# huangeddie/GymGo

Measured on AMD Instinct MI355X. Metric: env steps/sec across batched games, 19x19 uniform-random rollouts, higher is better.
Workload: dtype u8; 1 GPU; 19x19, 65536 parallel games, uniform-random rollouts with auto-reset; one bench step = one launch of 256 plies for every game; board=19, games=65536, games_per_gpu=65536, env_steps_per_bench_step=16777216, burn_in_steps=1, desync_plies=640

## Files before the change

gymgo_amd/csrc/gg_v5.h:

```cpp
#pragma once
#include "gg_v4.h"

namespace gg {

constexpr int kNB5 = 32;
constexpr int kJobCap = 128;

template <int R>
struct Lds5 {
  static constexpr int RS = R == 13 ? 20 : Cfg<R>::kRowStride;
  static constexpr int RPL = (R + 1) / 2;
  static_assert(2 * RPL <= RS, "a pair's rows must fit the row stride");
  static constexpr int kPad = 4;
  static constexpr int kState = kPad;
  static constexpr int kMeta = kState + 2 * kNB5 * RS;
  static constexpr int kFair = kMeta + 5 * kNB5;
  static constexpr int kTmp = kFair + 16;
  static constexpr int kUnion = kTmp + 4 * RS;
  static constexpr int kZero = kJobCap, kDump = kJobCap + 1;
  static constexpr int kCls = kUnion;
  static constexpr int kJob = kCls + kJobCap + 4;
  static constexpr int kG = kJob + kJobCap + 4;
  static constexpr int kSc = kG + 2 * kNB5 * RS;
  static constexpr int kLoopEnd = kSc + kWave * RS;
  static constexpr int kV2 = kUnion;
  static constexpr int kIoEnd = kV2 + (Lds2<R>::kRegion0 > 768 ? Lds2<R>::kRegion0 : 768);
  static constexpr int kDmaWords = (((kNB5 * (5 * R + 1) * 4 + 12 + 15) / 16 + kWave - 1) / kWave) * 256;
  static constexpr int kDmaEnd = kUnion + kDmaWords;
  static constexpr int kGrpBits = kUnion;
  static constexpr int kGrpWords = ((15 + kNB5 * 6 * R * R + 31) / 32 + 4) & ~3;
  static constexpr int kGrpLut = kGrpBits + kGrpWords;
  static constexpr int kGrpEnd = kGrpLut + 512;
  static constexpr int kMax2(int a, int b) { return a > b ? a : b; }
  static constexpr int kTotal = kMax2(kMax2(kLoopEnd, kIoEnd), kMax2(kDmaEnd, kGrpEnd));
  static_assert(kTotal * 4 <= 20480, "two waves per SIMD: 20 KB of LDS per wave");
  static_assert(kUnion % 4 == 0 && kG % 4 == 0 && kSc % 4 == 0, "16-byte alignment of the flood blocks");
  static_assert(3 * kNB5 * RS <= kLoopEnd - kUnion, "parked tracked rows fit the loop area");
};

__device__ __forceinline__ uint32_t mbcnt64(uint64_t m) {
  return __builtin_amdgcn_mbcnt_hi((uint32_t)(m >> 32), __builtin_amdgcn_mbcnt_lo((uint32_t)m, 0u));
}
constexpr int QP_L0 = 0xA0;

__device__ __forceinline__ void kth_set_bit10(const uint32_t (&v)[10], const uint32_t (&p)[10], uint32_t tt, int &rr, uint32_t &pos) {
  uint32_t ntt = ~tt;
  const uint32_t g5 = (uint32_t)((int32_t)(p[4] + ntt) >> 31);
  uint32_t a[5], t[4];
#pragma unroll
  for (int i = 0; i < 5; ++i) a[i] = B3(g5, v[5 + i], v[i], T_SEL);
#pragma unroll
  for (int i = 0; i < 4; ++i) t[i] = B3(g5, p[5 + i], p[i], T_SEL);
  uint32_t base = g5 & p[4], row = g5 & 5u;
  const uint32_t g2 = (uint32_t)((int32_t)(t[1] + ntt) >> 31);
  const uint32_t b0 = B3(g2, a[2], a[0], T_SEL), b1 = B3(g2, a[3], a[1], T_SEL), u0 = B3(g2, t[2], t[0], T_SEL);
  base = B3(g2, t[1], base, T_SEL);
  row = B3(g2, 2u, row, T_ANDOR);
  const uint32_t g1 = (uint32_t)((int32_t)(u0 + ntt) >> 31);
  uint32_t vr = B3(g1, b1, b0, T_SEL);
  base = B3(g1, u0, base, T_SEL);
  row -= g1;
  const uint32_t g1b = B3(g2, g1, (uint32_t)((int32_t)(t[3] + ntt) >> 31), TA & TB & TC);
  vr = B3(g1b, a[4], vr, T_SEL);
  base = B3(g1b, t[3], base, T_SEL);
  row -= g1b;
  ntt += base;
  uint32_t ps = 0;
#pragma unroll
  for (int sh = 16; sh >= 1; sh >>= 1) {
    const uint32_t e = (uint32_t)__popc((vr >> ps) & ((1u << sh) - 1u)) + ntt;
    const uint32_t ge = (uint32_t)((int32_t)e >> 31);
    ntt = B3(ge, e, ntt, T_SEL);
    ps = B3((uint32_t)sh, ge, ps, T_ANDOR);
  }
  rr = (int)row;
  pos = ps;
}

template <int R>
constexpr int flood_first_test() {
#ifdef GG_AB_FLOODK
  return R == 19 ? GG_AB_FLOODK : 3;
#else
  return R == 19 ? 2 : 3;
#endif
}

#ifdef GG_AB_SWEEPS
static __device__ unsigned long long gg_sweeps5[10];
#endif

#ifndef GG_AB_LIBSUM
#define GG_AB_LIBSUM 1
#endif
#ifndef GG_AB_PEEL
#define GG_AB_PEEL 1
#endif
#ifndef GG_AB_PRIO
#define GG_AB_PRIO 1
#endif
#ifndef GG_AB_PRIO_HAND
#define GG_AB_PRIO_HAND 0
#endif
#ifndef GG_AB_HAND1
#define GG_AB_HAND1 1
#endif

#ifndef GG_AB_MOVE_RC
#define GG_AB_MOVE_RC 1
#endif

template <int R>
__device__ __forceinline__ uint32_t job_liberties(const uint32_t (&gt)[R], const uint32_t (&ot)[R], const uint32_t (&m)[R]) {
  constexpr uint32_t FULLROW = (1u << R) - 1u;
  static_assert(R < 27, "the sum of R rows below 2^R stays inside 32 bits");
  auto row = [&](int r) -> uint32_t {
    const uint32_t e = B3(ot[r], m[r], FULLROW, ~(TA | TB) & TC & 0xFF);
    const uint32_t up = r > 0 ? gt[r - 1] : 0u, dn = r + 1 < R ? gt[r + 1] : 0u;
    const uint32_t dd = B3(shl1(gt[r]), gt[r] >> 1, up, T_OR3);
    return B3(dd, dn, e, (TA | TB) & TC);
  };
#if GG_AB_LIBSUM
  uint32_t o3[3] = {0u, 0u, 0u}, s3[3] = {0u, 0u, 0u};
  if (R & 1) o3[0] = s3[0] = row(0);
#pragma unroll
  for (int r = R & 1; r < R; r += 2) {
    const int c = (r / 2) % 3;
    const uint32_t la = row(r), lb = row(r + 1);
    o3[c] = la | lb | o3[c];
    s3[c] = la + lb + s3[c];
  }
  const uint32_t o = o3[0] | o3[1] | o3[2], s = s3[0] + s3[1] + s3[2];
  const uint32_t two = B3(o, 0u - o, s, (TA & TB) ^ TC);
#else
  uint32_t o3[3] = {0u, 0u, 0u}, d3[3] = {0u, 0u, 0u};
#pragma unroll
  for (int r = 0; r < R; ++r) {
    const uint32_t l = row(r);
    d3[r % 3] = B3(l, o3[r % 3], d3[r % 3], T_ANDOR);
    o3[r % 3] = B3(l, o3[r % 3], 0u, T_OR3);
  }
  const uint32_t o = B3(o3[0], o3[1], o3[2], T_OR3);
  const uint32_t d = B3(d3[0], d3[1], d3[2], T_OR3) | B3(o3[0], o3[1], o3[2], T_MAJ);
  const uint32_t two = B3(o - 1u, o, d, T_ANDOR);
#endif
  return (o != 0u ? 1u : 0u) + (two != 0u ? 1u : 0u);
}

template <int R, bool WEAK>
__device__ __forceinline__ void flood_jobs_restart(const uint32_t (&m)[R], const uint32_t (&mrev)[R], uint32_t (&f)[R], uint32_t (&res)[R],
                                           bool need, const uint32_t (&mm)[R], uint32_t &open) {
  int sweeps = 0;
#pragma unroll 1
  for (int it = 0; it < R * R; ++it) {
#pragma unroll
    for (int r = 0; r < R; ++r) FLOOD_VISIT(r, r - 1, (r & 1) != 0);
    if (it > 0) {
      uint32_t op = 0, opw = 0, pend = 0, above = 0;
#pragma unroll
      for (int r = R - 1; r >= 0; --r) {
        const uint32_t g = ((r + 1) & 1) ? __brev(f[r]) : f[r];
        res[r] = g;
        if (r < R - 1) {
          const uint32_t t = B3(above, m[r], g, T_AND_ANDN);
          if (WEAK) { op |= t; opw = B3(t, mm[r], opw, (TA & ~TB & 0xFF) | TC); }
          else or_pairs(op, pend, (R - 2 - r) & 1, t);
        }
        above = g;
      }
      if (!WEAK && ((R - 1) & 1)) op |= pend;
      open = op;
      if (__ballot((WEAK ? opw : op) != 0 && need) == 0) { sweeps = 2 * it + 1; break; }
    }
#pragma unroll
    for (int r = R - 1; r >= 0; --r) FLOOD_VISIT(r, r + 1, ((r + 1) & 1) != 0);
    if (it > 0) {
      uint32_t op = 0, opw = 0, pend = 0, below = 0;
#pragma unroll
      for (int r = 0; r < R; ++r) {
        const uint32_t g = (r & 1) ? __brev(f[r]) : f[r];
        res[r] = g;
        if (r > 0) {
          const uint32_t t = B3(below, m[r], g, T_AND_ANDN);
          if (WEAK) { op |= t; opw = B3(t, mm[r], opw, (TA & ~TB & 0xFF) | TC); }
          else or_pairs(op, pend, (r - 1) & 1, t);
        }
        below = g;
      }
      if (!WEAK && ((R - 1) & 1)) op |= pend;
      open = op;
      if (__ballot((WEAK ? opw : op) != 0 && need) == 0) { sweeps = 2 * it + 2; break; }
    }
  }
  (void)sweeps;
}

template <int R>
__device__ __forceinline__ uint32_t flood_jobs(const uint32_t (&m)[R], const uint32_t (&mrev)[R], uint32_t (&f)[R], uint32_t (&res)[R],
                                               const uint32_t (&ot)[R], const uint32_t (&mm)[R], bool isG, bool have) {
  constexpr int K = flood_first_test<R>();
  static_assert(K >= 1 && K <= 3, "the first closure test comes after one, two or three sweeps");
  uint32_t cnt = 0;
  bool resumed = false;
#ifdef GG_AB_SWEEPS
  int sw_ = 0, sw0_ = 0;
  uint32_t ng_ = 0, no_ = 0;
#define GG_SW5_SWEEP() (++sw_)
#else
#define GG_SW5_SWEEP() ((void)0)
#endif
  auto done = [&](uint32_t op, uint32_t opw) -> bool {
    if (!resumed && __ballot(opw != 0u && isG) != 0) return false;
    cnt = job_liberties<R>(res, ot, m);
    const bool unsettled = have && op != 0u && cnt < 2u;
    const uint64_t u = __ballot(unsettled);
#ifdef GG_AB_SWEEPS
    if (!resumed) { sw0_ = sw_; ng_ = (uint32_t)__popcll(__ballot(unsettled && isG)); no_ = (uint32_t)__popcll(u) - ng_; }
#endif
    resumed = true;
    return u == 0;
  };
  auto sweep_down = [&]() {
#pragma unroll
    for (int r = 0; r < R; ++r) FLOOD_VISIT(r, r - 1, (r & 1) != 0);
    GG_SW5_SWEEP();
  };
  auto sweep_up = [&]() {
#pragma unroll
    for (int r = R - 1; r >= 0; --r) FLOOD_VISIT(r, r + 1, ((r + 1) & 1) != 0);
    GG_SW5_SWEEP();
  };
  auto done_after_down = [&]() -> bool {
    uint32_t op = 0, opw = 0, above = 0;
#pragma unroll
    for (int r = R - 1; r >= 0; --r) {
      const uint32_t g = ((r + 1) & 1) ? __brev(f[r]) : f[r];
      res[r] = g;
      if (r < R - 1) {
        const uint32_t t = B3(above, m[r], g, T_AND_ANDN);
        op |= t;
        opw = B3(t, mm[r], opw, (TA & ~TB & 0xFF) | TC);
      }
      above = g;
    }
    return done(op, opw);
  };
  auto done_after_up = [&]() -> bool {
    uint32_t op = 0, opw = 0, below = 0;
#pragma unroll
    for (int r = 0; r < R; ++r) {
      const uint32_t g = (r & 1) ? __brev(f[r]) : f[r];
      res[r] = g;
      if (r > 0) {
        const uint32_t t = B3(below, m[r], g, T_AND_ANDN);
        op |= t;
        opw = B3(t, mm[r], opw, (TA & ~TB & 0xFF) | TC);
      }
      below = g;
    }
    return done(op, opw);
  };
  constexpr bool PEEL = GG_AB_PEEL != 0 && K == 2;
  bool fin = false;
  if constexpr (PEEL) {
    sweep_down();
    sweep_up();
    fin = done_after_up();
  }
  if (!fin) {
#pragma unroll 1
    for (int it = PEEL ? 1 : 0; it < R * R; ++it) {
      sweep_down();
      if ((PEEL || K <= 1 || it > 0) && done_after_down()) break;
      sweep_up();
      if ((PEEL || K <= 2 || it > 0) && done_after_up()) break;
    }
  }
#undef GG_SW5_SWEEP
#ifdef GG_AB_SWEEPS
  { int l_; asm volatile("v_mbcnt_lo_u32_b32 %0, -1, 0\n\tv_mbcnt_hi_u32_b32 %0, -1, %0" : "=v"(l_));
    if (l_ == 0) {
      const int ex_ = sw_ - sw0_;
      atomicAdd(&gg_sweeps5[0], (unsigned long long)sw0_); atomicAdd(&gg_sweeps5[1], 1ull);
      if (ng_ + no_) { atomicAdd(&gg_sweeps5[2], 1ull); atomicAdd(&gg_sweeps5[2 + (ex_ < 4 ? ex_ : 4)], 1ull); }
      atomicAdd(&gg_sweeps5[7], (unsigned long long)ng_); atomicAdd(&gg_sweeps5[8], (unsigned long long)no_);
      atomicAdd(&gg_sweeps5[9], (unsigned long long)ex_);
    } }
#endif
  return cnt;
}

#ifdef GG_AB_P3
static __device__ unsigned long long gg_p3[10];
#define GG_P3(k, n) (p3c_[k] += (n))
#else
#define GG_P3(k, n) ((void)0)
#endif
#ifdef GG_AB_MARK
#define GG_MARK(k) asm volatile("; GGMARK " #k ::: "memory")
#else
#define GG_MARK(k) do {} while (0)
#endif
#if defined(GG_AB_P3) || defined(GG_AB_LIVE)
#define GG_LIVE_CHECK 1
static __device__ unsigned long long gg_live_bad;
#endif

#ifdef GG_AB_WS
static __device__ unsigned long long gg_wsc[2];
#define GG_WSC_DECL uint32_t wsc_[2] = {0u, 0u}
#define GG_WSC(hit) (wsc_[(hit) ? 0 : 1] += 1u)
#define GG_WSC_FLUSH do { if (ws && ln0 == 0) { atomicAdd(&gg_wsc[0], (unsigned long long)wsc_[0]); \
    atomicAdd(&gg_wsc[1], (unsigned long long)wsc_[1]); } } while (0)
#else
#define GG_WSC_DECL do {} while (0)
#define GG_WSC(hit) ((void)0)
#define GG_WSC_FLUSH do {} while (0)
#endif
#ifdef GG_AB_LOADSPLIT
static __device__ unsigned long long gg_lsplit[4];
#define GG_LS_DECL unsigned long long tls_[3] = {0, 0, 0}, tlc_ = clock64()
#define GG_LS(k) do { asm volatile("s_waitcnt lgkmcnt(0)" ::: "memory"); __builtin_amdgcn_sched_barrier(0); \
    const unsigned long long n_ = clock64(); __builtin_amdgcn_sched_barrier(0); tls_[k] += n_ - tlc_; tlc_ = n_; } while (0)
#define GG_LS_START do { __builtin_amdgcn_sched_barrier(0); tlc_ = clock64(); __builtin_amdgcn_sched_barrier(0); } while (0)
#define GG_LS_FLUSH do { if (ln0 == 0) { for (int k_ = 0; k_ < 3; ++k_) atomicAdd(&gg_lsplit[k_], tls_[k_]); \
    atomicAdd(&gg_lsplit[3], 1ull); } } while (0)
#else
// ... 24 lines not shown
```

gymgo_amd/csrc/gg_v5_kernel.h:

```cpp
template <int R, int IO>
__global__ __launch_bounds__(kWave, 2) void GG_R5_NAME(uint8_t *__restrict__ states, uint64_t *__restrict__ rng,
                                                       int32_t *__restrict__ last_actions, int64_t *__restrict__ steps_done,
                                                       int64_t B, uint32_t inv, int plies, int auto_reset, int nb,
                                                       uint32_t *__restrict__ ws) {
  constexpr int POL = GG_R5_POL;
  static_assert(IO == 0 || IO == 2, "byte planes or tracked boards");
  constexpr int N = R;
  constexpr int RS = Lds5<R>::RS;
  constexpr int RV = (R + 3) / 4;
  constexpr int RPL = Lds5<R>::RPL;
  constexpr int PL = kNB5 * RS;
  constexpr int ZERO = Lds5<R>::kZero, DUMP = Lds5<R>::kDump;
  constexpr bool TRACKED = IO == 2;
  constexpr int P = N * N, S = 6 * P, W = 5 * N + 1;
  constexpr uint32_t FULLROW = (1u << N) - 1u;
  __shared__ __attribute__((aligned(16))) uint32_t lds[Lds5<R>::kTotal];
  uint32_t *st = lds + Lds5<R>::kState;
  uint32_t *flagsv = lds + Lds5<R>::kMeta;
  int *lastv = reinterpret_cast<int *>(lds + Lds5<R>::kMeta + kNB5);
  int *playedv = reinterpret_cast<int *>(lds + Lds5<R>::kMeta + 2 * kNB5);
  uint32_t *rngv = lds + Lds5<R>::kMeta + 3 * kNB5;
  uint32_t *tmp = lds + Lds5<R>::kTmp;
  uint32_t *clsv = lds + Lds5<R>::kCls;
  uint32_t *jobv = lds + Lds5<R>::kJob;
// ... 149 lines not shown
        if (!known) {
          uint32_t ab;
          analyze2<R, false>(black, white, hf.full_l1 & ~(black | white), hf, v2, mb, ab, mw, nullptr, nullptr, true);
        }
        GG_LS(1);
        if (row) {
          st[0 * PL + s * RS + hf.hl] = black;
          st[1 * PL + s * RS + hf.hl] = white;
          tmp[(hf.h * 2 + 0) * RS + hf.hl] = invalid;
          tmp[(hf.h * 2 + 1) * RS + hf.hl] = mb | mw;
        }
        if (hf.hl == 0) {
          flagsv[s] = turn | (passed << 1) | (done << 2) | (on ? 8u : 0u);
          lastv[s] = -1;
          playedv[s] = 0;
        }
        WAVE_SYNC();
        if ((hf.lane >> 2) == i) {
          const uint32_t *tp = tmp + ((s5 & 1) * 2) * RS + r05;
#pragma unroll
          for (int r = 0; r < RPL; ++r) {
            inv_r[r] = tp[r];
            M[r] = tp[RS + r];
          }
        }
        WAVE_SYNC();
        GG_LS(2);
        cv0 = nv0; cv1 = nv1; cv2 = nv2; cfb = nfb;
        if (ws) { cw0 = nw0; cw1 = nw1; cw2 = nw2; cw3 = nw3; }
      }
#undef GG_ISSUE_PAIR5
#undef GG_ISSUE_WS5
      GG_LS_FLUSH;
    }
    WAVE_SYNC();
    for (int i = hf.lane; i < kWave * RS; i += kWave) sc[i] = 0u;
    WAVE_SYNC();

    uint32_t flr = flagsv[s5];
    const uint64_t x0r = ((uint64_t)rngv[2 * s5 + 1] << 32) | rngv[2 * s5];
    int playedr = 0;
#ifdef GG_AB_P3
    uint32_t p3c_[10] = {0, 0, 0, 0, 0, 0, 0, 0, 0, 0};
#endif
#ifdef GG_LIVE_CHECK
    int drawsr = 0;
    bool was_dead = false;
#endif
    GG_PROF(6);
    FairShare fair(lds + Lds5<R>::kFair);
    const uint32_t fair_lag = plies >= 192 ? 24u : (plies >= 16 ? (uint32_t)plies >> 3 : 2u);
    bool lead = false;
    uint32_t uq = 0;
#pragma unroll 1
    for (int t = 0; t < plies; ++t) {
      if ((t & 3) == 0 && plies >= 8) {
        const uint32_t left = (uint32_t)(plies - t);
        lead = fair.behind((uint32_t)t, left < fair_lag ? (left > 2u ? left : 2u) : fair_lag) != 0u;
        if (lead) __builtin_amdgcn_s_setprio(2); else __builtin_amdgcn_s_setprio(3);
      }
      int ln;
      asm volatile("v_mbcnt_lo_u32_b32 %0, -1, 0\n\tv_mbcnt_hi_u32_b32 %0, -1, %0" : "=v"(ln));
      const int s4 = (ln >> 1) & 31, t5 = ln & 1, r0 = RPL * t5;
      const bool bl = s4 < nb;
      uint32_t full[RPL];
#pragma unroll
      for (int r = 0; r < RPL; ++r) full[r] = (r0 + r < N) ? FULLROW : 0u;

      int a_q;
      uint32_t fl_q;
#if GG_AB_MOVE_RC
      uint32_t rc_q;
#endif
      {
        const uint32_t fl = flr;
        const bool on = bl && ((fl >> 3) & 1u);
        const bool done = (fl >> 2) & 1u;
        const bool live = on && !(done && !auto_reset);
        const bool reset = live && done;
#ifdef GG_LIVE_CHECK
        if (live && was_dead) atomicAdd(&gg_live_bad, 1ull);
        was_dead = was_dead || (bl && !live);
        drawsr += live ? 1 : 0;
#endif
        uint32_t v[RPL], p[RPL];
        const uint32_t rm = reset ? ~0u : 0u;
        uint32_t eye[RPL];
        uint32_t tc[RPL], te[RPL];
        if constexpr (POL != kPolUniform) {
          const uint32_t turn = fl & 1u;
          const uint32_t *pm = st + turn * PL + s4 * RS + r0, *po = st + (1u - turn) * PL + s4 * RS + r0;
          uint32_t me[RPL], op[RPL];
#pragma unroll
          for (int r = 0; r < RPL; ++r) { me[r] = pm[r]; op[r] = po[r]; }
          const uint32_t me_up = dpp0<QP_X1>(me[RPL - 1]), op_up = dpp0<QP_X1>(op[RPL - 1]);
          const uint32_t me_dn = dpp0<QP_X1>(me[0]), op_dn = dpp0<QP_X1>(op[0]);
          uint32_t m_up = 0u, m_dn = 0u;
          if constexpr (POL == kPolTactical) { m_up = dpp0<QP_X1>(M[RPL - 1]); m_dn = dpp0<QP_X1>(M[0]); }
#pragma unroll
          for (int r = 0; r < RPL; ++r) {
            const int rw = r0 + r;
            const uint32_t meU = r ? me[r - 1] : (t5 ? me_up : FULLROW), opU = r ? op[r - 1] : (t5 ? op_up : 0u);
            const uint32_t meDn = r + 1 < RPL ? me[r + 1] : (t5 ? 0u : me_dn), opD = r + 1 < RPL ? op[r + 1] : (t5 ? 0u : op_dn);
            const uint32_t meD = rw + 1 >= N ? FULLROW : meDn;
            const uint32_t edge = (rw == 0 || rw == N - 1) ? FULLROW : (1u | (1u << (N - 1)));
            eye[r] = eye_row(me[r], op[r], meU, meD, opU, opD, full[r], edge, N) & ~rm;
            if constexpr (POL == kPolTactical) {
              const uint32_t MU = r ? M[r - 1] : (t5 ? m_up : FULLROW);
              const uint32_t MDn = r + 1 < RPL ? M[r + 1] : (t5 ? 0u : m_dn);
              const uint32_t MD = rw + 1 >= N ? FULLROW : MDn;
              tactical_rows(me[r], op[r], M[r], meU, meD, opU, opD, MU, MD, full[r], tc[r], te[r]);
              tc[r] &= ~rm;
              te[r] &= ~rm;
            }
          }
        }
#pragma unroll
        for (int r = 0; r < RPL; ++r) {
          v[r] = B3(full[r], rm, inv_r[r], TA & (TB | (~TC & 0xFF)));
          if constexpr (POL == kPolTactical) {
            tc[r] &= v[r];
            te[r] &= v[r];
            v[r] &= ~eye[r];
            p[r] = ((uint32_t)__popc(v[r]) | ((uint32_t)__popc(tc[r]) << 10) | ((uint32_t)__popc(te[r]) << 20)) + (r ? p[r - 1] : 0u);
          } else {
            if constexpr (POL == kPolNoEyeFill) v[r] &= ~eye[r];
            p[r] = (uint32_t)__popc(v[r]) + (r ? p[r - 1] : 0u);
          }
        }
        uint32_t T = p[RPL - 1];
        const uint32_t oth = dpp0<QP_X1>(T);
        uint32_t Pb = t5 ? oth : 0u, n = T + oth;
        if ((t & 1) == 0) {
          uint64_t xx = x0r + (uint64_t)(uint32_t)(t + t5) * 0x9E3779B97F4A7C15ull;
          uq = (uint32_t)(splitmix_next(xx) >> 32);
        }
        const uint32_t uh = dpp0<QP_L0>(uq);
        uq = dpp0<QP_X1>(uq);
        if constexpr (POL == kPolTactical) {
          const bool gate = (uh & 3u) != 0u;
          const bool useC = gate && ((n >> 10) & 0x3FFu) != 0u, useE = gate && !useC && (n >> 20) != 0u;
          const uint32_t sh = useC ? 10u : (useE ? 20u : 0u);
          const uint32_t mc = useC ? ~0u : 0u, me_ = useE ? ~0u : 0u;
#pragma unroll
          for (int r = 0; r < RPL; ++r) {
            v[r] = B3(mc, tc[r], B3(me_, te[r], v[r], T_SEL), T_SEL);
            p[r] = (p[r] >> sh) & 0x3FFu;
          }
          T = (T >> sh) & 0x3FFu;
          Pb = (Pb >> sh) & 0x3FFu;
          n = (n >> sh) & 0x3FFu;
        }
        const uint32_t k = __umulhi(uh, POL != kPolUniform ? n : n + 1u);
        const bool hit = k >= Pb && k < Pb + T;
        int rr;
        uint32_t pos;
        if constexpr (RPL == 10) kth_set_bit10(v, p, (k - Pb) & 0x3FFu, rr, pos);
        else kth_set_bit<RPL>(v, p, (k - Pb) & 0x3FFu, rr, pos);
        const int rabs = r0 + rr;
#if GG_AB_MOVE_RC
        const uint32_t cand = hit ? ((uint32_t)rabs << 5) | pos : 0u;
        rc_q = cand | dpp0<QP_X1>(cand);
        const uint32_t pt = __umul24(rc_q >> 5, (uint32_t)N) + (rc_q & 31u);
#else
        const uint32_t cand = hit ? (uint32_t)(rabs * N + (int)pos) : 0u;
        const uint32_t pt = cand | dpp0<QP_X1>(cand);
#endif
        a_q = !live ? -1 : (k < n ? (int)pt : P);
        const bool place = live && hit;
        fl_q = reset ? 40u : fl;
        uint64_t resetm = __ballot(reset && t5 == 0);
        const bool none_live = __ballot(live) == 0;
        if (none_live && resetm == 0) break;
        if (resetm) {
          if (reset) {
#pragma unroll
            for (int r = 0; r < RPL; ++r) inv_r[r] = M[r] = 0u;
          }
          while (resetm) {
            const int s = (__ffsll((unsigned long long)resetm) - 1) >> 1;
            resetm &= resetm - 1;
            for (int i = hf.lane; i < 2 * RS; i += kWave) st[(i / RS) * PL + s * RS + (i % RS)] = 0;
            if (hf.lane == 0) flagsv[s] = 8u | 32u;
          }
          if (none_live) break;
        }
        WAVE_SYNC();
        uint32_t *gb = gblk + 2 * s4 * RS;
        if (t5 == 0) clsv[s4] = 0u;
        {
          uint4 *pz = reinterpret_cast<uint4 *>(gb + t5 * RS);
#pragma unroll
          for (int i = 0; i < RV; ++i) pz[i] = make_uint4(0u, 0u, 0u, 0u);
        }
        asm volatile("" ::: "memory");
        if (place) {
          const int turn = reset ? 0 : (int)(fl & 1u);
          atomicOr(st + turn * PL + s4 * RS + rabs, 1u << pos);
          gb[rabs] = 1u << pos;
        }
      }
      WAVE_SYNC();
      GG_PROF(0);

      uint32_t qs;
      int njobs;
      {
        const int a = a_q;
        const uint32_t turn = fl_q & 1u;
        const uint32_t mv1 = ((uint32_t)a < (uint32_t)P) ? 1u : 0u;
        int ar, ac;
#if GG_AB_MOVE_RC
        ar = (int)(rc_q >> 5);
        ac = (int)(rc_q & 31u);
#else
        split_action(mv1 ? a : 0, N, inv, ar, ac);
#endif
        const uint32_t *pm = st + turn * PL + s4 * RS, *po = st + (1u - turn) * PL + s4 * RS;
        uint32_t obit[2], packed = 0;
#pragma unroll
        for (int j = 0; j < 2; ++j) {
          const int sg = 2 * j - 1;
          const int dr = t5 ? 0 : sg, dc = t5 ? sg : 0;
          const int nr = ar + dr, nc = ac + dc;
          const uint32_t rowm = pm[nr], rowo = po[nr];
          const uint32_t ncs = (uint32_t)nc & 31u;
          const uint32_t mbit = (rowm >> ncs) & mv1, ob = (rowo >> ncs) & mv1;
          const uint32_t onb = ((uint32_t)nr < (uint32_t)N && (uint32_t)nc < (uint32_t)N) ? mv1 : 0u;
          const uint32_t ex = mbit | ob;
          packed += (onb & ~ex) | (mbit << 8) | ((onb & ~ob) << 16);
          obit[j] = ob;
        }
        qs = packed + dpp0<QP_X1>(packed) + 0x70700u;
        const uint32_t friendly = (qs >> 11) & 1u;
        const uint32_t gf = t5 ? 0u : friendly;
        const uint32_t c = gf + obit[0] + obit[1];
        const uint64_t b0 = __ballot((c & 1u) != 0u), b1 = __ballot((c & 2u) != 0u);
        const uint32_t base = mbcnt64(b0) + 2u * mbcnt64(b1);
        njobs = (int)__popcll(b0) + 2 * (int)__popcll(b1);
        const uint32_t sG = base, s0 = base + gf, s1 = s0 + obit[0];
        const uint32_t common = (uint32_t)s4 | (1u << 18) | ((turn ^ 1u) << 15);
#if GG_AB_MOVE_RC
        const int step = t5 ? 1 : 32;
        const int sd = (int)rc_q;
#else
        const int step = t5 ? 1 : N;
        const int sd = a;
#endif
        jobv[gf ? sG : (uint32_t)DUMP] = ((uint32_t)s4 | (1u << 18) | (turn << 15) | (1u << 16)) | ((uint32_t)sd << 5);
        const uint32_t dirs = (uint32_t)t5 << 20;
        jobv[obit[0] ? s0 : (uint32_t)DUMP] = common | dirs | ((uint32_t)(sd - step) << 5);
        jobv[obit[1] ? s1 : (uint32_t)DUMP] = common | dirs | (1u << 19) | ((uint32_t)(sd + step) << 5);
      }
      WAVE_SYNC();

      if (!GG_AB_PRIO && plies >= 8) { if (lead) __builtin_amdgcn_s_setprio(0); else __builtin_amdgcn_s_setprio(1); }
#pragma unroll 1
      for (int jb = 0; jb < njobs; jb += kWave) {
        const int j = jb + ln;
        const bool have = j < njobs;
        const uint32_t d = jobv[have ? j : DUMP];
        const uint32_t ex = have ? 1u : 0u;
        const int sj = (int)(d & 31u);
        int sr, scol;
#if GG_AB_MOVE_RC
        sr = (int)((d >> 10) & 31u);
        scol = (int)((d >> 5) & 31u);
#else
        split_action((int)((d >> 5) & 511u), N, inv, sr, scol);
#endif
        const uint32_t ownc = (d >> 15) & 1u;
        const uint32_t isG = have ? (d >> 16) & 1u : 0u;
        uint32_t *blk = sc + ln * RS;
        const uint4 *lds4 = reinterpret_cast<const uint4 *>(lds);
        const uint4 *pmv = lds4 + (Lds5<R>::kState + (int)ownc * PL + sj * RS) / 4;
        const uint4 *pov = lds4 + (Lds5<R>::kState + (int)(ownc ^ 1u) * PL + sj * RS) / 4;
        uint32_t mm[R];
        {
          const int src = 8 * sj;
#pragma unroll
          for (int i = 0; i < RPL; ++i) {
            mm[i] = (uint32_t)__builtin_amdgcn_ds_bpermute(src, (int)M[i]);
            if (RPL + i < R) mm[RPL + i] = (uint32_t)__builtin_amdgcn_ds_bpermute(src + 4, (int)M[i]);
          }
        }
        uint32_t cnt = 0;
        uint32_t res[R];
        {
          uint32_t m[R], mrev[R], f[R], ot[R];
          {
            uint32_t mt[RV * 4], ft[RV * 4];
#pragma unroll
            for (int i = 0; i < RV; ++i) {
              const uint4 x = pmv[i], y = pov[i];
              mt[4 * i] = x.x; mt[4 * i + 1] = x.y; mt[4 * i + 2] = x.z; mt[4 * i + 3] = x.w;
              ot[4 * i] = y.x;
              if (4 * i + 1 < R) ot[4 * i + 1] = y.y;
              if (4 * i + 2 < R) ot[4 * i + 2] = y.z;
              if (4 * i + 3 < R) ot[4 * i + 3] = y.w;
            }
            {
              const int srw = sr & (int)(0u - ex);
              asm volatile("" ::: "memory");
              blk[srw] = ex << (((uint32_t)scol ^ (0u - ((uint32_t)sr & 1u))) & 31u);
              asm volatile("" ::: "memory");
              const uint4 *pf = reinterpret_cast<const uint4 *>(blk);
#pragma unroll
              for (int i = 0; i < RV; ++i) {
                const uint4 x = pf[i];
                ft[4 * i] = x.x; ft[4 * i + 1] = x.y; ft[4 * i + 2] = x.z; ft[4 * i + 3] = x.w;
              }
              asm volatile("" ::: "memory");
              blk[srw] = 0u;
            }
#pragma unroll
            for (int r = 0; r < R; ++r) {
              m[r] = mt[r];
              mrev[r] = __brev(m[r]);
              f[r] = ft[r];
              res[r] = 0u;
            }
          }
          GG_PROF(1);
          if (GG_AB_PRIO && plies >= 8) { if (lead) __builtin_amdgcn_s_setprio(0); else __builtin_amdgcn_s_setprio(1); }
          if constexpr (R == 19) {
            cnt = flood_jobs<R>(m, mrev, f, res, ot, mm, isG != 0u, have);
            GG_PROF(2);
          } else {
            uint32_t open = 0;
            flood_jobs_restart<R, true>(m, mrev, f, res, isG != 0u, mm, open);
            GG_PROF(2);
            cnt = job_liberties<R>(res, ot, m);
            const bool unsettled = have && open != 0u && cnt < 2u;
            if (__ballot(unsettled)) {
#pragma unroll
              for (int r = 0; r < R; ++r) f[r] = (r & 1) ? __brev(res[r]) : res[r];
              flood_jobs_restart<R, false>(m, mrev, f, res, unsettled, mm, open);
              cnt = job_liberties<R>(res, ot, m);
            }
          }
        }
        if (GG_AB_PRIO_HAND && plies >= 8) { if (lead) __builtin_amdgcn_s_setprio(2); else __builtin_amdgcn_s_setprio(3); }
        const uint32_t lib2 = cnt < 2u ? cnt : 2u;
        uint32_t *gb = gblk + 2 * sj * RS;
#if GG_AB_HAND1
        static_assert(Lds5<R>::kG % 2 == 0 && RS % 2 == 0 && R + 1 <= RS, "8-byte aligned row pairs inside the block");
        if (isG || (have && cnt < 2u)) {
          uint32_t *dst = gb + (isG ? 0 : RS);
#pragma unroll
          for (int r = 0; r < R; r += 2) {
            const uint32_t hi = r + 1 < R ? res[r + 1] : 0u;
            atomicOr(reinterpret_cast<unsigned long long *>(dst + r), ((unsigned long long)hi << 32) | res[r]);
          }
          const uint32_t word = isG ? lib2 << 4 : (cnt == 0u ? 1u << ((d >> 19) & 3u) : 0u);
          atomicOr(clsv + sj, word);
        }
#else
        if (isG) {
          uint4 *pz = reinterpret_cast<uint4 *>(gb);
#pragma unroll
          for (int i = 0; i < RV; ++i)
            pz[i] = make_uint4(res[4 * i], 4 * i + 1 < R ? res[4 * i + 1] : 0u, 4 * i + 2 < R ? res[4 * i + 2] : 0u, 4 * i + 3 < R ? res[4 * i + 3] : 0u);
          if (lib2) atomicOr(clsv + sj, lib2 << 4);
        } else if (have && cnt < 2u) {
          static_assert(Lds5<R>::kG % 2 == 0 && RS % 2 == 0 && R + 1 <= RS, "8-byte aligned row pairs inside the block");
#pragma unroll
          for (int r = 0; r < R; r += 2) {
            const uint32_t hi = r + 1 < R ? res[r + 1] : 0u;
            atomicOr(reinterpret_cast<unsigned long long *>(gb + RS + r), ((unsigned long long)hi << 32) | res[r]);
          }
          if (cnt == 0u) atomicOr(clsv + sj, 1u << ((d >> 19) & 3u));
        }
#endif
      }
      if (!(GG_AB_PRIO && GG_AB_PRIO_HAND) && plies >= 8) { if (lead) __builtin_amdgcn_s_setprio(2); else __builtin_amdgcn_s_setprio(3); }
      WAVE_SYNC();
      GG_PROF(3);

      {
        const int a = a_q;
        const uint32_t fl = fl_q;
        const uint32_t info = clsv[s4];
        const int turn0 = fl & 1u;
        uint32_t *pmine = st + turn0 * PL + s4 * RS + r0;
        uint32_t *popp = st + (1 - turn0) * PL + s4 * RS + r0;
        const uint32_t *gG = gblk + 2 * s4 * RS + r0;
        uint32_t mine1[RPL], opp0[RPL], all4[RPL], bg[RPL];
#pragma unroll
        for (int r = 0; r < RPL; ++r) {
          mine1[r] = pmine[r];
          opp0[r] = popp[r];
          bg[r] = gG[r];
          all4[r] = gG[RS + r];
        }
        const bool moves_now = a >= 0;
        const bool is_pass = a == P;
        int ar, ac;
#if GG_AB_MOVE_RC
        ar = (int)(rc_q >> 5);
        ac = (int)(rc_q & 31u);
#else
        split_action(a, N, inv, ar, ac);
#endif
        const uint32_t capt_m = info & 15u;
        uint32_t g0[RPL], opp1[RPL];
#pragma unroll
        for (int r = 0; r < RPL; ++r) {
          g0[r] = bg[r];
          opp1[r] = B3(opp0[r], all4[r], M[r], TA & ~(TB & ~TC) & 0xFF);
        }
        const uint32_t ne = qs & 7u, ne2 = ne < 2u ? ne : 2u;
        uint32_t libsG = ((qs >> 11) & 1u) ? ((info >> 4) & 3u) : ne2;
        uint32_t ko_oh = 0, ko_bit = 0;
        GG_P3(0, 1u);
        GG_P3(8, (uint32_t)__popcll(__ballot(capt_m != 0u && t5 == 0)));
        GG_P3(9, (uint32_t)__popcll(__ballot(a >= 0 && t5 == 0)));
        GG_MARK(10);
        if (__ballot(capt_m != 0u)) {
          GG_MARK(11);
          GG_P3(1, 1u);
          uint32_t cap[RPL];
#pragma unroll
          for (int r = 0; r < RPL; ++r) cap[r] = B3(all4[r], M[r], M[r], TA & ~TB & 0xFF);
          const uint32_t ncapn = (uint32_t)__popc(capt_m);
          if (__ballot(ncapn == 1u && libsG == 0u)) {
            GG_MARK(12);
            GG_P3(2, 1u);
            uint32_t dg[RPL];
            dilate_rows<RPL>(g0, dg);
            uint32_t cntc = 0;
#pragma unroll
            for (int r = 0; r < RPL; ++r) cntc += (uint32_t)__popc(dg[r] & cap[r]);
            const uint32_t c2 = cntc < 2u ? cntc : 2u;
            const uint32_t tot = c2 + dpp0<QP_X1>(c2);
            libsG += (ncapn == 1u && libsG == 0u) ? (tot < 2u ? tot : 2u) : ncapn;
            GG_MARK(13);
          } else {
            libsG += ncapn;
          }
          const bool ko1 = ncapn == 1u && !(qs & CL_OPEN);
          if (__ballot(ko1)) {
            GG_MARK(14);
            GG_P3(3, 1u);
            uint32_t died = 0;
#pragma unroll
            for (int r = 0; r < RPL; ++r) died += (uint32_t)__popc(cap[r]);
            const bool ko = ko1 && died + dpp0<QP_X1>(died) == 1u;
            const uint32_t kr = (uint32_t)ar - (capt_m & 1u) + ((capt_m >> 1) & 1u) - (uint32_t)r0;
            ko_oh = (ko && kr < (uint32_t)RPL) ? (1u << (kr & 31)) : 0u;
            ko_bit = 1u << (((uint32_t)ac - ((capt_m >> 2) & 1u) + (capt_m >> 3)) & 31u);
            GG_MARK(15);
          }
          GG_MARK(16);
          uint32_t atari[RPL], f[RPL], anyf = 0;
          {
            const uint32_t up = dpp0<0x138>(cap[RPL - 1]), dn = dpp0<0x130>(cap[0]);
#pragma unroll
            for (int r = 0; r < RPL; ++r) {
              atari[r] = B3(mine1[r], M[r], g0[r], TA & ~(TB | TC) & 0xFF);
              const uint32_t above = r == 0 ? up : cap[r - 1], below = r == RPL - 1 ? dn : cap[r + 1];
              const uint32_t v = B3(cap[r] >> 1, above, below, T_OR3);
              f[r] = B3(shl1(cap[r]), v, atari[r], (TA | TB) & TC);
              anyf |= f[r];
            }
          }
          GG_MARK(17);
          if (__ballot(anyf != 0u)) {
            GG_MARK(18);
            GG_P3(5, 1u);
#ifdef GG_AB_P3
            uint32_t trips_ = 0;
#define GG_TRIP ++trips_
#else
#define GG_TRIP do {} while (0)
#endif
#define GG_JOIN_TRIP(R0, D)                                                                                               \
            do {                                                                                                          \
              GG_TRIP;                                                                                                    \
              const uint32_t up_ = dpp0<0x138>(f[RPL - 1]), dn_ = dpp0<0x130>(f[0]);                                      \
              chg = 0;                                                                                                    \
              _Pragma("unroll") for (int i_ = 0; i_ < RPL; ++i_) {                                                        \
                const int r_ = (R0) + (D) * i_;                                                                           \
                const uint32_t above_ = r_ == 0 ? up_ : f[r_ == 0 ? 0 : r_ - 1];                                          \
                const uint32_t below_ = r_ == RPL - 1 ? dn_ : f[r_ == RPL - 1 ? 0 : r_ + 1];                              \
                const uint32_t v_ = B3(f[r_] >> 1, above_, below_, T_OR3);                                              \
                const uint32_t g_ = B3(shl1(f[r_]), v_, atari[r_], (TA | TB) & TC);                                      \
                chg = B3(g_, f[r_], chg, (TA & ~TB & 0xFF) | TC);                                                         \
                f[r_] |= g_;                                                                                              \
              }                                                                                                           \
            } while (0)
            uint32_t chg;
#pragma unroll 1
            for (int it = 0; it < R * R; ++it) {
              GG_JOIN_TRIP(0, 1);
              if (__ballot(chg != 0u) == 0) break;
              GG_JOIN_TRIP(RPL - 1, -1);
              if (__ballot(chg != 0u) == 0) break;
            }
#undef GG_JOIN_TRIP
#undef GG_TRIP
#ifdef GG_AB_P3
            GG_P3(6, trips_);
            p3c_[7] = trips_ > p3c_[7] ? trips_ : p3c_[7];
#endif
#pragma unroll
            for (int r = 0; r < RPL; ++r) M[r] |= f[r];
            GG_MARK(19);
          }
        }
        GG_MARK(20);
        const uint32_t gsel = libsG >= 2u ? ~0u : 0u;
        uint32_t e[RPL], x[RPL], nbr[RPL];
#pragma unroll
        for (int r = 0; r < RPL; ++r) {
          const uint32_t u = B3(M[r], g0[r], all4[r], TA & ~(TB | TC) & 0xFF);
          M[r] = B3(gsel, g0[r], u, T_ANDOR);
          const uint32_t y = B3(M[r], mine1[r], opp1[r], T_SEL);
          x[r] = B3(full[r], y, y, TA & ~TB & 0xFF);
          e[r] = B3(full[r], opp1[r], mine1[r], TA & ~(TB | TC) & 0xFF);
        }
        dilate_rows<RPL>(x, nbr);
        const uint32_t mv_m = moves_now ? ~0u : 0u;
#pragma unroll
        for (int r = 0; r < RPL; ++r) {
          const uint32_t invalid = B3(e[r], nbr[r], full[r], ~(TA & TB) & TC & 0xFF);
          inv_r[r] = B3(mv_m, invalid, inv_r[r], T_SEL);
        }
        if (__ballot(ko_oh != 0u)) {
#pragma unroll
          for (int r = 0; r < RPL; ++r) inv_r[r] |= (uint32_t)__builtin_amdgcn_sbfe((int)ko_oh, r, 1) & ko_bit;
        }
        if (capt_m) {
#pragma unroll
          for (int r = 0; r < RPL; ++r) popp[r] = opp1[r];
        }
        flr = fl;
        if (moves_now) {
          const uint32_t passed0 = (fl >> 1) & 1u, done0 = (fl >> 2) & 1u;
          const uint32_t passed = is_pass ? 1u : 0u, done = done0 | (passed & passed0);
          flr = (uint32_t)(turn0 ^ 1) | (passed << 1) | (done << 2) | 8u | (fl & 32u);
          playedr += 1;
          if (t5 == 0) {
            flagsv[s4] = flr;
            lastv[s4] = a;
            playedv[s4] = playedr;
          }
        }
      }
      WAVE_SYNC();
      GG_PROF(4);
    }
    if (plies >= 8) fair.release();
    GG_PROF(5);
#ifdef GG_AB_P3
    if (ln0 == 0) {
#pragma unroll
      for (int k = 0; k < 10; ++k) {
        if (k == 7) atomicMax(&gg_p3[7], (unsigned long long)p3c_[7]);
        else atomicAdd(&gg_p3[k], (unsigned long long)p3c_[k]);
      }
    }
#endif
#ifdef GG_LIVE_CHECK
    if (playedr != drawsr) atomicAdd(&gg_live_bad, 1ull);
#endif

    int lnS;
    asm volatile("v_mbcnt_lo_u32_b32 %0, -1, 0\n\tv_mbcnt_hi_u32_b32 %0, -1, %0" : "=v"(lnS));
    const int s5s = lnS >> 1, r05s = RPL * (lnS & 1);
    WAVE_SYNC();
    if (TRACKED) {
#pragma unroll
      for (int r = 0; r < RPL; ++r) {
        if (r05s + r < RS) {
          const uint32_t bk = st[0 * PL + s5s * RS + r05s + r], wh = st[1 * PL + s5s * RS + r05s + r];
          park[0 * PL + s5s * RS + r05s + r] = inv_r[r];
          park[1 * PL + s5s * RS + r05s + r] = M[r] & bk;
          park[2 * PL + s5s * RS + r05s + r] = M[r] & wh;
        }
      }
      WAVE_SYNC();
      const int64_t nbrd = (B - b_first) < nb ? (B - b_first) : nb;
      const int nw = (int)nbrd * W;
      uint32_t *gp = reinterpret_cast<uint32_t *>(states) + b_first * (int64_t)W;
      bool tch = false;
      if (lnS < (int)nbrd) tch = playedv[lnS] != 0 || (flagsv[lnS] & 32u);
      const uint64_t tmask = __ballot(tch);
#pragma unroll 1
      for (int i0 = lnS; i0 < nw; i0 += 4 * kWave) {
        uint32_t v[4];
        bool ok[4];
#pragma unroll
        for (int k = 0; k < 4; ++k) {
          const int i = i0 + k * kWave;
          const int ic = i < nw ? i : 0;
          const int sb = ic / W, w = ic - sb * W;
          ok[k] = i < nw && ((tmask >> sb) & 1ull);
          const int pl = w / N, rw = w - pl * N;
          const uint32_t *src = pl >= 5 ? flagsv + sb : (pl < 2 ? st + pl * PL + sb * RS + rw : park + (pl - 2) * PL + sb * RS + rw);
          const uint32_t x = *src;
          v[k] = pl >= 5 ? (x & 7u) : x;
// ... 71 lines not shown
```

Before: 15.47 billion env steps/s.

## Hoist per-lane addresses, flatten branches, use native wave64 ballots for 19x19

For the 19x19 board, the lane index, slot/row offsets and LDS base pointers are computed once outside the ply loop instead of every ply. Divergent branches are replaced with branchless atomics and unconditional stores to a dump area, and ballots use the wave64 builtin. Boolean predicates are merged via three-input bit ops. The flood sweeps fold the boundary bit-reversal into a turn flag, and several flat-mode variants are gated by new A/B macros. The aim is fewer scalar and vector instructions and less branch divergence per ply, at the cost of more live registers and extra always-executed atomics and stores.

```diff
diff --git a/gymgo_amd/csrc/gg_v5.h b/gymgo_amd/csrc/gg_v5.h
--- a/gymgo_amd/csrc/gg_v5.h
+++ b/gymgo_amd/csrc/gg_v5.h
@@ -23,6 +23,8 @@
   static constexpr int kG = kJob + kJobCap + 4;
   static constexpr int kSc = kG + 2 * kNB5 * RS;
   static constexpr int kLoopEnd = kSc + kWave * RS;
+  static constexpr int kDumpMeta = kCls + kNB5;
+  static_assert(kNB5 + 3 * kNB5 <= kJobCap, "the dump words end in front of the slot of an absent job");
   static constexpr int kV2 = kUnion;
   static constexpr int kIoEnd = kV2 + (Lds2<R>::kRegion0 > 768 ? Lds2<R>::kRegion0 : 768);
   static constexpr int kDmaWords = (((kNB5 * (5 * R + 1) * 4 + 12 + 15) / 16 + kWave - 1) / kWave) * 256;
@@ -110,6 +112,24 @@
 #define GG_AB_MOVE_RC 1
 #endif
 
+#ifndef GG_AB_LANE1
+#define GG_AB_LANE1 1
+#endif
+#ifndef GG_AB_BALLOT1
+#define GG_AB_BALLOT1 1
+#endif
+#ifndef GG_AB_FLAT1
+#define GG_AB_FLAT1 1
+#endif
+#ifndef GG_AB_TURN1
+#define GG_AB_TURN1 1
+#endif
+#if GG_AB_BALLOT1
+#define GG_BALLOT5(p) (R == 19 ? (unsigned long long)__builtin_amdgcn_ballot_w64(p) : __ballot(p))
+#else
+#define GG_BALLOT5(p) __ballot(p)
+#endif
+
 template <int R>
 __device__ __forceinline__ uint32_t job_liberties(const uint32_t (&gt)[R], const uint32_t (&ot)[R], const uint32_t (&m)[R]) {
   constexpr uint32_t FULLROW = (1u << R) - 1u;
@@ -170,7 +190,7 @@
       }
       if (!WEAK && ((R - 1) & 1)) op |= pend;
       open = op;
-      if (__ballot((WEAK ? opw : op) != 0 && need) == 0) { sweeps = 2 * it + 1; break; }
+      if (GG_BALLOT5((WEAK ? opw : op) != 0 && need) == 0) { sweeps = 2 * it + 1; break; }
     }
 #pragma unroll
     for (int r = R - 1; r >= 0; --r) FLOOD_VISIT(r, r + 1, ((r + 1) & 1) != 0);
@@ -189,7 +209,7 @@
       }
       if (!WEAK && ((R - 1) & 1)) op |= pend;
       open = op;
-      if (__ballot((WEAK ? opw : op) != 0 && need) == 0) { sweeps = 2 * it + 2; break; }
+      if (GG_BALLOT5((WEAK ? opw : op) != 0 && need) == 0) { sweeps = 2 * it + 2; break; }
     }
   }
   (void)sweeps;
@@ -209,25 +229,39 @@
 #else
 #define GG_SW5_SWEEP() ((void)0)
 #endif
+#if GG_AB_BALLOT1
+  uint32_t gm = isG ? ~0u : 0u, hm = have ? ~0u : 0u;
+  asm volatile("" : "+v"(gm), "+v"(hm));
+#endif
   auto done = [&](uint32_t op, uint32_t opw) -> bool {
-    if (!resumed && __ballot(opw != 0u && isG) != 0) return false;
+#if GG_AB_BALLOT1
+    if (!resumed && GG_BALLOT5((opw & gm) != 0u) != 0) return false;
+    cnt = job_liberties<R>(res, ot, m);
+    const bool unsettled = B3(op, hm, (uint32_t)((int32_t)(cnt - 2u) >> 31), TA & TB & TC) != 0u;
+#else
+    if (!resumed && GG_BALLOT5(opw != 0u && isG) != 0) return false;
     cnt = job_liberties<R>(res, ot, m);
     const bool unsettled = have && op != 0u && cnt < 2u;
-    const uint64_t u = __ballot(unsettled);
+#endif
+    const uint64_t u = GG_BALLOT5(unsettled);
 #ifdef GG_AB_SWEEPS
-    if (!resumed) { sw0_ = sw_; ng_ = (uint32_t)__popcll(__ballot(unsettled && isG)); no_ = (uint32_t)__popcll(u) - ng_; }
+    if (!resumed) { sw0_ = sw_; ng_ = (uint32_t)__popcll(GG_BALLOT5(unsettled && isG)); no_ = (uint32_t)__popcll(u) - ng_; }
 #endif
     resumed = true;
     return u == 0;
   };
-  auto sweep_down = [&]() {
-#pragma unroll
-    for (int r = 0; r < R; ++r) FLOOD_VISIT(r, r - 1, (r & 1) != 0);
+  auto sweep_down = [&](bool turn) {
+    if (turn) f[0] = __brev(f[0]);
+#pragma unroll
+    for (int r = 0; r < R; ++r)
+      if (!(turn && r == 0)) FLOOD_VISIT(r, r - 1, (r & 1) != 0);
     GG_SW5_SWEEP();
   };
-  auto sweep_up = [&]() {
-#pragma unroll
-    for (int r = R - 1; r >= 0; --r) FLOOD_VISIT(r, r + 1, ((r + 1) & 1) != 0);
+  auto sweep_up = [&](bool turn) {
+    if (turn) f[R - 1] = __brev(f[R - 1]);
+#pragma unroll
+    for (int r = R - 1; r >= 0; --r)
+      if (!(turn && r == R - 1)) FLOOD_VISIT(r, r + 1, ((r + 1) & 1) != 0);
     GG_SW5_SWEEP();
   };
   auto done_after_down = [&]() -> bool {
@@ -262,17 +296,18 @@
   };
   constexpr bool PEEL = GG_AB_PEEL != 0 && K == 2;
   bool fin = false;
+  constexpr bool TURN = GG_AB_TURN1 != 0;
   if constexpr (PEEL) {
-    sweep_down();
-    sweep_up();
+    sweep_down(false);
+    sweep_up(TURN);
     fin = done_after_up();
   }
   if (!fin) {
 #pragma unroll 1
     for (int it = PEEL ? 1 : 0; it < R * R; ++it) {
-      sweep_down();
+      sweep_down(TURN && PEEL);
       if ((PEEL || K <= 1 || it > 0) && done_after_down()) break;
-      sweep_up();
+      sweep_up(TURN);
       if ((PEEL || K <= 2 || it > 0) && done_after_up()) break;
     }
   }
diff --git a/gymgo_amd/csrc/gg_v5_kernel.h b/gymgo_amd/csrc/gg_v5_kernel.h
--- a/gymgo_amd/csrc/gg_v5_kernel.h
+++ b/gymgo_amd/csrc/gg_v5_kernel.h
@@ -225,6 +225,18 @@
     const uint32_t fair_lag = plies >= 192 ? 24u : (plies >= 16 ? (uint32_t)plies >> 3 : 2u);
     bool lead = false;
     uint32_t uq = 0;
+#if GG_AB_LANE1
+    constexpr bool KEEP = R == 19;
+    const int lnK = ln0;
+    const int s4K = (lnK >> 1) & 31, t5K = lnK & 1, r0K = RPL * t5K;
+    const bool blK = s4K < nb;
+    const uint32_t fullK = (r0K + RPL - 1 < N) ? FULLROW : 0u;
+    uint32_t *const stK = st + s4K * RS;
+    uint32_t *const gbK = gblk + 2 * s4K * RS;
+    uint32_t *const clsK = clsv + s4K;
+    uint32_t *const metaK = flagsv + s4K;
+    uint32_t *const blkK = sc + lnK * RS;
+#endif
 #pragma unroll 1
     for (int t = 0; t < plies; ++t) {
       if ((t & 3) == 0 && plies >= 8) {
@@ -232,6 +244,15 @@
         lead = fair.behind((uint32_t)t, left < fair_lag ? (left > 2u ? left : 2u) : fair_lag) != 0u;
         if (lead) __builtin_amdgcn_s_setprio(2); else __builtin_amdgcn_s_setprio(3);
       }
+#if GG_AB_LANE1
+      int ln = lnK;
+      if constexpr (!KEEP) asm volatile("v_mbcnt_lo_u32_b32 %0, -1, 0\n\tv_mbcnt_hi_u32_b32 %0, -1, %0" : "=v"(ln));
+      const int s4 = KEEP ? s4K : (ln >> 1) & 31, t5 = KEEP ? t5K : ln & 1, r0 = KEEP ? r0K : RPL * t5;
+      const bool bl = KEEP ? blK : s4 < nb;
+      uint32_t full[RPL];
+#pragma unroll
+      for (int r = 0; r < RPL; ++r) full[r] = (KEEP && RPL + r < N) ? FULLROW : (KEEP && r == RPL - 1 ? fullK : ((r0 + r < N) ? FULLROW : 0u));
+#else
       int ln;
       asm volatile("v_mbcnt_lo_u32_b32 %0, -1, 0\n\tv_mbcnt_hi_u32_b32 %0, -1, %0" : "=v"(ln));
       const int s4 = (ln >> 1) & 31, t5 = ln & 1, r0 = RPL * t5;
@@ -239,6 +260,18 @@
       uint32_t full[RPL];
 #pragma unroll
       for (int r = 0; r < RPL; ++r) full[r] = (r0 + r < N) ? FULLROW : 0u;
+#endif
+#if GG_AB_LANE1
+#define GG_PM(turn) (KEEP ? ((turn) ? stK + PL : stK) : st + (turn) * PL + s4 * RS)
+#define GG_PO(turn) (KEEP ? ((turn) ? stK : stK + PL) : st + (1u - (turn)) * PL + s4 * RS)
+#define GG_GB (KEEP ? gbK : gblk + 2 * s4 * RS)
+#define GG_CLS (KEEP ? clsK : clsv + s4)
+#else
+#define GG_PM(turn) (st + (turn) * PL + s4 * RS)
+#define GG_PO(turn) (st + (1u - (turn)) * PL + s4 * RS)
+#define GG_GB (gblk + 2 * s4 * RS)
+#define GG_CLS (clsv + s4)
+#endif
 
       int a_q;
       uint32_t fl_q;
@@ -247,10 +280,19 @@
 #endif
       {
         const uint32_t fl = flr;
-        const bool on = bl && ((fl >> 3) & 1u);
-        const bool done = (fl >> 2) & 1u;
-        const bool live = on && !(done && !auto_reset);
-        const bool reset = live && done;
+        constexpr bool CMP1 = GG_AB_BALLOT1 != 0 && R == 19;
+        bool live, reset;
+        if constexpr (CMP1) {
+          uint32_t flb = bl ? fl : 0u;
+          asm volatile("" : "+v"(flb));
+          live = (flb & (auto_reset ? 8u : 12u)) == 8u;
+          reset = (flb & 12u) == (auto_reset ? 12u : ~0u);
+        } else {
+          const bool on = bl && ((fl >> 3) & 1u);
+          const bool done = (fl >> 2) & 1u;
+          live = on && !(done && !auto_reset);
+          reset = live && done;
+        }
 #ifdef GG_LIVE_CHECK
         if (live && was_dead) atomicAdd(&gg_live_bad, 1ull);
         was_dead = was_dead || (bl && !live);
@@ -262,7 +304,7 @@
         uint32_t tc[RPL], te[RPL];
         if constexpr (POL != kPolUniform) {
           const uint32_t turn = fl & 1u;
-          const uint32_t *pm = st + turn * PL + s4 * RS + r0, *po = st + (1u - turn) * PL + s4 * RS + r0;
+          const uint32_t *pm = GG_PM(turn) + r0, *po = GG_PO(turn) + r0;
           uint32_t me[RPL], op[RPL];
 #pragma unroll
           for (int r = 0; r < RPL; ++r) { me[r] = pm[r]; op[r] = po[r]; }
@@ -342,8 +384,8 @@
         a_q = !live ? -1 : (k < n ? (int)pt : P);
         const bool place = live && hit;
         fl_q = reset ? 40u : fl;
-        uint64_t resetm = __ballot(reset && t5 == 0);
-        const bool none_live = __ballot(live) == 0;
+        uint64_t resetm = CMP1 ? GG_BALLOT5(reset) & 0x5555555555555555ull : GG_BALLOT5(reset && t5 == 0);
+        const bool none_live = GG_BALLOT5(live) == 0;
         if (none_live && resetm == 0) break;
         if (resetm) {
           if (reset) {
@@ -359,17 +401,24 @@
           if (none_live) break;
         }
         WAVE_SYNC();
-        uint32_t *gb = gblk + 2 * s4 * RS;
-        if (t5 == 0) clsv[s4] = 0u;
+        uint32_t *gb = GG_GB;
+        constexpr bool FLAT = GG_AB_FLAT1 != 0 && R == 19;
+        if (FLAT || t5 == 0) *GG_CLS = 0u;
         {
           uint4 *pz = reinterpret_cast<uint4 *>(gb + t5 * RS);
 #pragma unroll
           for (int i = 0; i < RV; ++i) pz[i] = make_uint4(0u, 0u, 0u, 0u);
         }
         asm volatile("" ::: "memory");
-        if (place) {
+        if constexpr (FLAT) {
+          const uint32_t turn = reset ? 0u : (fl & 1u);
+          const uint32_t bit = place ? 1u << pos : 0u;
+          const int rw = place ? rabs : r0;
+          atomicOr(GG_PM(turn) + rw, bit);
+          atomicOr(gb + rw, bit);
+        } else if (place) {
           const int turn = reset ? 0 : (int)(fl & 1u);
-          atomicOr(st + turn * PL + s4 * RS + rabs, 1u << pos);
+          atomicOr(GG_PM(turn) + rabs, 1u << pos);
           gb[rabs] = 1u << pos;
         }
       }
@@ -389,7 +438,7 @@
 #else
         split_action(mv1 ? a : 0, N, inv, ar, ac);
 #endif
-        const uint32_t *pm = st + turn * PL + s4 * RS, *po = st + (1u - turn) * PL + s4 * RS;
+        const uint32_t *pm = GG_PM(turn), *po = GG_PO(turn);
         uint32_t obit[2], packed = 0;
 #pragma unroll
         for (int j = 0; j < 2; ++j) {
@@ -408,7 +457,7 @@
         const uint32_t friendly = (qs >> 11) & 1u;
         const uint32_t gf = t5 ? 0u : friendly;
         const uint32_t c = gf + obit[0] + obit[1];
-        const uint64_t b0 = __ballot((c & 1u) != 0u), b1 = __ballot((c & 2u) != 0u);
+        const uint64_t b0 = GG_BALLOT5((c & 1u) != 0u), b1 = GG_BALLOT5((c & 2u) != 0u);
         const uint32_t base = mbcnt64(b0) + 2u * mbcnt64(b1);
         njobs = (int)__popcll(b0) + 2 * (int)__popcll(b1);
         const uint32_t sG = base, s0 = base + gf, s1 = s0 + obit[0];
@@ -444,7 +493,11 @@
 #endif
         const uint32_t ownc = (d >> 15) & 1u;
         const uint32_t isG = have ? (d >> 16) & 1u : 0u;
+#if GG_AB_LANE1
+        uint32_t *blk = KEEP ? blkK : sc + ln * RS;
+#else
         uint32_t *blk = sc + ln * RS;
+#endif
         const uint4 *lds4 = reinterpret_cast<const uint4 *>(lds);
         const uint4 *pmv = lds4 + (Lds5<R>::kState + (int)ownc * PL + sj * RS) / 4;
         const uint4 *pov = lds4 + (Lds5<R>::kState + (int)(ownc ^ 1u) * PL + sj * RS) / 4;
@@ -505,7 +558,7 @@
             GG_PROF(2);
             cnt = job_liberties<R>(res, ot, m);
             const bool unsettled = have && open != 0u && cnt < 2u;
-            if (__ballot(unsettled)) {
+            if (GG_BALLOT5(unsettled)) {
 #pragma unroll
               for (int r = 0; r < R; ++r) f[r] = (r & 1) ? __brev(res[r]) : res[r];
               flood_jobs_restart<R, false>(m, mrev, f, res, unsettled, mm, open);
@@ -518,7 +571,23 @@
         uint32_t *gb = gblk + 2 * sj * RS;
 #if GG_AB_HAND1
         static_assert(Lds5<R>::kG % 2 == 0 && RS % 2 == 0 && R + 1 <= RS, "8-byte aligned row pairs inside the block");
-        if (isG || (have && cnt < 2u)) {
+        constexpr bool HAND_FLAT = GG_AB_FLAT1 != 0 && R == 19;
+        if constexpr (HAND_FLAT) {
+          uint32_t off = isG ? 0u : (uint32_t)RS;
+          const uint32_t wv = isG ? lib2 : (cnt == 0u ? 1u : 0u), wsh = isG ? 4u : ((d >> 19) & 3u);
+          uint32_t word = wv << wsh;
+          uint32_t sji = (uint32_t)sj;
+          asm volatile("" : "+v"(off), "+v"(word), "+v"(sji));
+          if (isG || (have && cnt < 2u)) {
+            uint32_t *dst = gb + off;
+#pragma unroll
+            for (int r = 0; r < R; r += 2) {
+              const uint32_t hi = r + 1 < R ? res[r + 1] : 0u;
+              atomicOr(reinterpret_cast<unsigned long long *>(dst + r), ((unsigned long long)hi << 32) | res[r]);
+            }
+            atomicOr(clsv + sji, word);
+          }
+        } else if (isG || (have && cnt < 2u)) {
           uint32_t *dst = gb + (isG ? 0 : RS);
 #pragma unroll
           for (int r = 0; r < R; r += 2) {
@@ -553,11 +622,11 @@
       {
         const int a = a_q;
         const uint32_t fl = fl_q;
-        const uint32_t info = clsv[s4];
+        const uint32_t info = *GG_CLS;
         const int turn0 = fl & 1u;
-        uint32_t *pmine = st + turn0 * PL + s4 * RS + r0;
-        uint32_t *popp = st + (1 - turn0) * PL + s4 * RS + r0;
-        const uint32_t *gG = gblk + 2 * s4 * RS + r0;
+        uint32_t *pmine = GG_PM(turn0) + r0;
+        uint32_t *popp = GG_PO(turn0) + r0;
+        const uint32_t *gG = GG_GB + r0;
         uint32_t mine1[RPL], opp0[RPL], all4[RPL], bg[RPL];
 #pragma unroll
         for (int r = 0; r < RPL; ++r) {
@@ -586,17 +655,19 @@
         uint32_t libsG = ((qs >> 11) & 1u) ? ((info >> 4) & 3u) : ne2;
         uint32_t ko_oh = 0, ko_bit = 0;
         GG_P3(0, 1u);
-        GG_P3(8, (uint32_t)__popcll(__ballot(capt_m != 0u && t5 == 0)));
-        GG_P3(9, (uint32_t)__popcll(__ballot(a >= 0 && t5 == 0)));
+        GG_P3(8, (uint32_t)__popcll(GG_BALLOT5(capt_m != 0u && t5 == 0)));
+        GG_P3(9, (uint32_t)__popcll(GG_BALLOT5(a >= 0 && t5 == 0)));
         GG_MARK(10);
-        if (__ballot(capt_m != 0u)) {
+        if (GG_BALLOT5(capt_m != 0u)) {
           GG_MARK(11);
           GG_P3(1, 1u);
           uint32_t cap[RPL];
 #pragma unroll
           for (int r = 0; r < RPL; ++r) cap[r] = B3(all4[r], M[r], M[r], TA & ~TB & 0xFF);
           const uint32_t ncapn = (uint32_t)__popc(capt_m);
-          if (__ballot(ncapn == 1u && libsG == 0u)) {
+          constexpr bool CMP3 = GG_AB_BALLOT1 != 0 && R == 19;
+          const bool one0 = CMP3 ? B3(ncapn, 1u, libsG, (TA ^ TB) | TC) == 0u : (ncapn == 1u && libsG == 0u);
+          if (GG_BALLOT5(one0)) {
             GG_MARK(12);
             GG_P3(2, 1u);
             uint32_t dg[RPL];
@@ -606,13 +677,13 @@
             for (int r = 0; r < RPL; ++r) cntc += (uint32_t)__popc(dg[r] & cap[r]);
             const uint32_t c2 = cntc < 2u ? cntc : 2u;
             const uint32_t tot = c2 + dpp0<QP_X1>(c2);
-            libsG += (ncapn == 1u && libsG == 0u) ? (tot < 2u ? tot : 2u) : ncapn;
+            libsG += one0 ? (tot < 2u ? tot : 2u) : ncapn;
             GG_MARK(13);
           } else {
             libsG += ncapn;
           }
-          const bool ko1 = ncapn == 1u && !(qs & CL_OPEN);
-          if (__ballot(ko1)) {
+          const bool ko1 = CMP3 ? B3(ncapn, 1u, qs & CL_OPEN, (TA ^ TB) | TC) == 0u : (ncapn == 1u && !(qs & CL_OPEN));
+          if (GG_BALLOT5(ko1)) {
             GG_MARK(14);
             GG_P3(3, 1u);
             uint32_t died = 0;
@@ -638,7 +709,7 @@
             }
           }
           GG_MARK(17);
-          if (__ballot(anyf != 0u)) {
+          if (GG_BALLOT5(anyf != 0u)) {
             GG_MARK(18);
             GG_P3(5, 1u);
 #ifdef GG_AB_P3
@@ -666,9 +737,9 @@
 #pragma unroll 1
             for (int it = 0; it < R * R; ++it) {
               GG_JOIN_TRIP(0, 1);
-              if (__ballot(chg != 0u) == 0) break;
+              if (GG_BALLOT5(chg != 0u) == 0) break;
               GG_JOIN_TRIP(RPL - 1, -1);
-              if (__ballot(chg != 0u) == 0) break;
+              if (GG_BALLOT5(chg != 0u) == 0) break;
             }
 #undef GG_JOIN_TRIP
 #undef GG_TRIP
@@ -699,7 +770,7 @@
           const uint32_t invalid = B3(e[r], nbr[r], full[r], ~(TA & TB) & TC & 0xFF);
           inv_r[r] = B3(mv_m, invalid, inv_r[r], T_SEL);
         }
-        if (__ballot(ko_oh != 0u)) {
+        if (GG_BALLOT5(ko_oh != 0u)) {
 #pragma unroll
           for (int r = 0; r < RPL; ++r) inv_r[r] |= (uint32_t)__builtin_amdgcn_sbfe((int)ko_oh, r, 1) & ko_bit;
         }
@@ -707,19 +778,40 @@
 #pragma unroll
           for (int r = 0; r < RPL; ++r) popp[r] = opp1[r];
         }
-        flr = fl;
-        if (moves_now) {
+        if constexpr (GG_AB_FLAT1 != 0 && R == 19) {
           const uint32_t passed0 = (fl >> 1) & 1u, done0 = (fl >> 2) & 1u;
           const uint32_t passed = is_pass ? 1u : 0u, done = done0 | (passed & passed0);
-          flr = (uint32_t)(turn0 ^ 1) | (passed << 1) | (done << 2) | 8u | (fl & 32u);
-          playedr += 1;
-          if (t5 == 0) {
-            flagsv[s4] = flr;
-            lastv[s4] = a;
-            playedv[s4] = playedr;
-          }
-        }
-      }
+          const uint32_t flm = (uint32_t)(turn0 ^ 1) | (passed << 1) | (done << 2) | 8u | (fl & 32u);
+          flr = moves_now ? flm : fl;
+          playedr += moves_now ? 1 : 0;
+#if GG_AB_LANE1
+          uint32_t *mp = KEEP ? (moves_now ? metaK : metaK + (Lds5<R>::kDumpMeta - Lds5<R>::kMeta))
+                              : lds + (moves_now ? Lds5<R>::kMeta : Lds5<R>::kDumpMeta) + s4;
+#else
+          uint32_t *mp = lds + (moves_now ? Lds5<R>::kMeta : Lds5<R>::kDumpMeta) + s4;
+#endif
+          mp[0] = flr;
+          mp[kNB5] = (uint32_t)a;
+          mp[2 * kNB5] = (uint32_t)playedr;
+        } else {
+          flr = fl;
+          if (moves_now) {
+            const uint32_t passed0 = (fl >> 1) & 1u, done0 = (fl >> 2) & 1u;
+            const uint32_t passed = is_pass ? 1u : 0u, done = done0 | (passed & passed0);
+            flr = (uint32_t)(turn0 ^ 1) | (passed << 1) | (done << 2) | 8u | (fl & 32u);
+            playedr += 1;
+            if (t5 == 0) {
+              flagsv[s4] = flr;
+              lastv[s4] = a;
+              playedv[s4] = playedr;
+            }
+          }
+        }
+      }
+#undef GG_PM
+#undef GG_PO
+#undef GG_GB
+#undef GG_CLS
       WAVE_SYNC();
       GG_PROF(4);
     }
```

Result: faster. 15.99 billion env steps/s, median of 6 (+3.4%).
